# orottier/web-audio-api-rs

Measured on NVIDIA H100. Metric: offline render-quanta/sec (48kHz stereo, 128-frame), higher is better.
Workload: dtype f64 filter state / f32 PCM

## Files before the change

web-audio-api-rs_b200/csrc/wae_kernels.cu:

```cuda
#include "wae_kernels.h"
#include "wae_param_core.h"
#include "wae_param_walk.h"
#include "../../include/wae.h"

#include <algorithm>
#include <cmath>
#include <cstdlib>
#include <vector>
#include <type_traits>
#include <cuda_runtime.h>
#include <math_constants.h>

namespace wae {

#define DEVI __device__ __forceinline__

DEVI float* chan(const BufRef& b, int c, const ChunkInfo& ci) { return b.p + (size_t)c * b.stride + (b.absolute ? ci.f0 : ci.sub); }

DEVI int meta_qi(const ChunkInfo& ci, int n) { return (ci.sub + n) >> 7; }
DEVI bool buf_silent(const BufRef& b, int rows, int qi) {
    if (!b.meta) return false;
    for (int r = 0; r < rows; r++)
        if (!(b.meta[(size_t)r * b.meta_stride + qi] & WAE_META_SILENT)) return false;
    return true;
// ... 3366 lines not shown
    u = cadd(a[2], a[6]); v = csub(a[2], a[6]); a[2] = u; a[6] = cmul(rot16<4>(v, sign), t1);
    u = cadd(a[3], a[7]); v = csub(a[3], a[7]); a[3] = u; a[7] = cmul(rot16<6>(v, sign), t1);
#pragma unroll
    for (int g = 0; g < 8; g += 4) {
        u = cadd(a[g], a[g + 2]); v = csub(a[g], a[g + 2]); a[g] = u; a[g + 2] = cmul(v, t2);
        u = cadd(a[g + 1], a[g + 3]); v = csub(a[g + 1], a[g + 3]); a[g + 1] = u; a[g + 3] = cmul(rot16<4>(v, sign), t2);
    }
#pragma unroll
    for (int m = 0; m < 8; m += 2) {
        u = cadd(a[m], a[m + 1]); v = csub(a[m], a[m + 1]); a[m] = u; a[m + 1] = cmul(v, t3);
    }
}
WAE_HD void bf8_dit(float2 (&a)[8], float2 t1, int sign) {
    const float2 t2 = cmul(t1, t1), t3 = cmul(t2, t2);
    float2 u, v;
#pragma unroll
    for (int m = 0; m < 8; m += 2) {
        v = cmul(a[m + 1], t3); u = a[m]; a[m] = cadd(u, v); a[m + 1] = csub(u, v);
    }
#pragma unroll
    for (int g = 0; g < 8; g += 4) {
        v = cmul(a[g + 2], t2); u = a[g]; a[g] = cadd(u, v); a[g + 2] = csub(u, v);
        v = rot16<4>(cmul(a[g + 3], t2), sign); u = a[g + 1]; a[g + 1] = cadd(u, v); a[g + 3] = csub(u, v);
    }
    v = cmul(a[4], t1); u = a[0]; a[0] = cadd(u, v); a[4] = csub(u, v);
    v = rot16<2>(cmul(a[5], t1), sign); u = a[1]; a[1] = cadd(u, v); a[5] = csub(u, v);
    v = rot16<4>(cmul(a[6], t1), sign); u = a[2]; a[2] = cadd(u, v); a[6] = csub(u, v);
    v = rot16<6>(cmul(a[7], t1), sign); u = a[3]; a[3] = cadd(u, v); a[7] = csub(u, v);
}
WAE_HD void bf16_dif(float2 (&a)[16], int sign) {
    float2 u, v;
#define WAE_BF(i, j, M) u = cadd(a[i], a[j]); v = csub(a[i], a[j]); a[i] = u; a[j] = rot16<M>(v, sign);
    WAE_BF(0, 8, 0) WAE_BF(1, 9, 1) WAE_BF(2, 10, 2) WAE_BF(3, 11, 3) WAE_BF(4, 12, 4) WAE_BF(5, 13, 5) WAE_BF(6, 14, 6) WAE_BF(7, 15, 7)
#pragma unroll
    for (int g = 0; g < 16; g += 8) {
        WAE_BF(g, g + 4, 0) WAE_BF(g + 1, g + 5, 2) WAE_BF(g + 2, g + 6, 4) WAE_BF(g + 3, g + 7, 6)
    }
#pragma unroll
    for (int g = 0; g < 16; g += 4) {
        WAE_BF(g, g + 2, 0) WAE_BF(g + 1, g + 3, 4)
    }
#pragma unroll
    for (int g = 0; g < 16; g += 2) {
        WAE_BF(g, g + 1, 0)
    }
#undef WAE_BF
}
WAE_HD void bf16_dit(float2 (&a)[16], int sign) {
    float2 u, v;
#define WAE_BF(i, j, M) v = rot16<M>(a[j], sign); u = a[i]; a[i] = cadd(u, v); a[j] = csub(u, v);
#pragma unroll
    for (int g = 0; g < 16; g += 2) {
        WAE_BF(g, g + 1, 0)
    }
#pragma unroll
    for (int g = 0; g < 16; g += 4) {
        WAE_BF(g, g + 2, 0) WAE_BF(g + 1, g + 3, 4)
    }
#pragma unroll
    for (int g = 0; g < 16; g += 8) {
        WAE_BF(g, g + 4, 0) WAE_BF(g + 1, g + 5, 2) WAE_BF(g + 2, g + 6, 4) WAE_BF(g + 3, g + 7, 6)
    }
    WAE_BF(0, 8, 0) WAE_BF(1, 9, 1) WAE_BF(2, 10, 2) WAE_BF(3, 11, 3) WAE_BF(4, 12, 4) WAE_BF(5, 13, 5) WAE_BF(6, 14, 6) WAE_BF(7, 15, 7)
#undef WAE_BF
}
struct FftTw { float2 w1, w2, w3; };
static_assert(CV_THREADS == 256 && CV_LOGB == 13, "FftTw assumes 4 radix-8 butterflies per thread and spans 1024 / 128 / 16");
WAE_HD FftTw fft_tw_of(const float2* tw, int t, int sign) {
    FftTw w;
    w.w1 = tw[t << 1];
    w.w2 = tw[(t & 127) << 4];
    w.w3 = tw[(t & 15) << 7];
    if (sign > 0) w.w1.y = -w.w1.y, w.w2.y = -w.w2.y, w.w3.y = -w.w3.y;
    return w;
}
WAE_HD float2 tw_it(float2 w1, int it, int sign) {
    float c, s;
    if (it == 0) return w1;
    if (it == 1) c = 0.98078528040323044913f, s = 0.19509032201612826785f;
    else if (it == 2) c = 0.92387953251128675613f, s = 0.38268343236508977173f;
    else c = 0.83146961230254523708f, s = 0.55557023301960222474f;
    return cmul(w1, make_float2(c, sign > 0 ? s : -s));
}
template <int LOG_Q, bool DIT>
WAE_HD void fft_pass8_one(float2* s, int t, int it, const FftTw& w, int sign) {
    constexpr int q = 1 << LOG_Q;
    const int bf = t + it * CV_THREADS;
    const int lo = bf & (q - 1), hi = bf >> LOG_Q;
    const int base = (hi << (LOG_Q + 3)) + lo;
    float2 a[8];
#pragma unroll
    for (int m = 0; m < 8; m++) a[m] = s[cv_pad(base + m * q)];
    const float2 t1 = LOG_Q == 10 ? tw_it(w.w1, it, sign) : (LOG_Q == 7 ? w.w2 : w.w3);
    if (DIT) bf8_dit(a, t1, sign);
    else bf8_dif(a, t1, sign);
#pragma unroll
    for (int m = 0; m < 8; m++) s[cv_pad(base + m * q)] = a[m];
}
template <bool DIT>
WAE_HD void fft_pass16_one(float2* s, int t, int it, int sign) {
    float2 a[16];
    float2* p = s + cv_pad((t + it * CV_THREADS) * 16);
#pragma unroll
    for (int m = 0; m < 16; m++) a[m] = p[m];
    if (DIT) bf16_dit(a, sign);
    else bf16_dif(a, sign);
#pragma unroll
    for (int m = 0; m < 16; m++) p[m] = a[m];
}
#ifndef WAE_CV_UNROLL
#define WAE_CV_UNROLL 2
#endif
template <int LOG_Q, bool DIT>
DEVI void fft_pass8(float2* s, const FftTw& w, int sign) {
#pragma unroll 1
    for (int i0 = 0; i0 < CV_B / 8 / CV_THREADS; i0 += WAE_CV_UNROLL) {
#pragma unroll
        for (int u = 0; u < WAE_CV_UNROLL; u++) fft_pass8_one<LOG_Q, DIT>(s, threadIdx.x, i0 + u, w, sign);
    }
}
template <bool DIT>
DEVI void fft_pass16(float2* s, int sign) {
#pragma unroll 1
    for (int it = 0; it < CV_B / 16 / CV_THREADS; it++) fft_pass16_one<DIT>(s, threadIdx.x, it, sign);
}
DEVI FftTw fft_tw_load(int sign) { return fft_tw_of(c_tw, threadIdx.x, sign); }
DEVI void fft_dif_smem(float2* s, const FftTw& w) {
    fft_pass8<10, false>(s, w, -1);
    __syncthreads();
    fft_pass8<7, false>(s, w, -1);
    __syncthreads();
    fft_pass8<4, false>(s, w, -1);
    __syncthreads();
    fft_pass16<false>(s, -1);
    __syncthreads();
}
DEVI void fft_dit_smem(float2* s, const FftTw& w) {
    fft_pass16<true>(s, +1);
    __syncthreads();
    fft_pass8<4, true>(s, w, +1);
    __syncthreads();
    fft_pass8<7, true>(s, w, +1);
    __syncthreads();
    fft_pass8<10, true>(s, w, +1);
    __syncthreads();
}
DEVI float2 cv_lane_tw() { return c_tw[cv_brev(threadIdx.x & 31)]; }
DEVI float2 cv_bin_tw(float2 lane_tw, int p) { return cmul(lane_tw, c_rowtw[p >> 5]); }
WAE_HD int cv_mirror(int p) { return cv_brev(CV_B - cv_brev(p)); }
WAE_HD float2 rfft_split(float2 zk, float2 zm, float2 tw) {
    const float2 zc = make_float2(zm.x, -zm.y);
    const float2 e = make_float2(0.5f * (zk.x + zc.x), 0.5f * (zk.y + zc.y));
    const float2 d = make_float2(zk.x - zc.x, zk.y - zc.y);
    const float2 o = make_float2(0.5f * d.y, -0.5f * d.x);
    const float2 r = cmul(tw, o);
    return make_float2(e.x + r.x, e.y + r.y);
}
WAE_HD float2 irfft_merge(float2 yk, float2 ym, float2 tw) {
    const float2 yc = make_float2(ym.x, -ym.y);
    const float2 e = make_float2(yk.x + yc.x, yk.y + yc.y);
    const float2 d = make_float2(yk.x - yc.x, yk.y - yc.y);
    const float2 o = cmul(make_float2(tw.x, -tw.y), d);
    return make_float2(e.x - o.y, e.y + o.x);
}
DEVI void rfft_store(const float2* z, float2* __restrict__ X, float2 lane_tw) {
#pragma unroll 4
    for (int p = threadIdx.x; p < CV_B; p += CV_THREADS) {
        float2 r;
        if (p == 0) {
            const float2 z0 = z[0];
            r = make_float2(z0.x + z0.y, z0.x - z0.y);
        } else {
            r = rfft_split(z[cv_pad(p)], z[cv_pad(cv_mirror(p))], cv_bin_tw(lane_tw, p));
        }
        X[p] = r;
    }
}
DEVI void conv_load_half(float2* z, int c0, const float* __restrict__ src, int valid, const float* __restrict__ src2 = nullptr) {
    const int t = threadIdx.x;
    if (!src || valid <= 0) {
        for (int i = t; i < CV_B / 2; i += CV_THREADS) z[cv_pad(c0 + i)] = make_float2(0.f, 0.f);
    } else if (src2 && ((reinterpret_cast<uintptr_t>(src) | reinterpret_cast<uintptr_t>(src2)) & 15) == 0) {
#pragma unroll 8
        for (int i4 = t; i4 < CV_B / 4; i4 += CV_THREADS) {
            const int n = 4 * i4;
            float4 v = make_float4(0.f, 0.f, 0.f, 0.f);
            if (n + 3 < valid) {
                const float4 a = *reinterpret_cast<const float4*>(src + n), c = *reinterpret_cast<const float4*>(src2 + n);
                v = make_float4(0.5f * (a.x + c.x), 0.5f * (a.y + c.y), 0.5f * (a.z + c.z), 0.5f * (a.w + c.w));
            } else if (n < valid) {
                v.x = 0.5f * (src[n] + src2[n]);
                if (n + 1 < valid) v.y = 0.5f * (src[n + 1] + src2[n + 1]);
                if (n + 2 < valid) v.z = 0.5f * (src[n + 2] + src2[n + 2]);
            }
            float2* d = z + cv_pad(c0 + 2 * i4);
            d[0] = make_float2(v.x, v.y);
            d[1] = make_float2(v.z, v.w);
        }
    } else if (src2) {
        for (int i = t; i < CV_B / 2; i += CV_THREADS) {
            const int n = 2 * i;
            z[cv_pad(c0 + i)] = make_float2(n < valid ? 0.5f * (src[n] + src2[n]) : 0.f, n + 1 < valid ? 0.5f * (src[n + 1] + src2[n + 1]) : 0.f);
        }
    } else if ((reinterpret_cast<uintptr_t>(src) & 15) == 0) {
#pragma unroll 8
        for (int i4 = t; i4 < CV_B / 4; i4 += CV_THREADS) {
            const int n = 4 * i4;
            float4 v = make_float4(0.f, 0.f, 0.f, 0.f);
            if (n + 3 < valid) v = *reinterpret_cast<const float4*>(src + n);
            else if (n < valid) {
                v.x = src[n];
                if (n + 1 < valid) v.y = src[n + 1];
                if (n + 2 < valid) v.z = src[n + 2];
            }
            float2* d = z + cv_pad(c0 + 2 * i4);
            d[0] = make_float2(v.x, v.y);
            d[1] = make_float2(v.z, v.w);
        }
    } else {
        for (int i = t; i < CV_B / 2; i += CV_THREADS) {
            const int n = 2 * i;
            z[cv_pad(c0 + i)] = make_float2(n < valid ? src[n] : 0.f, n + 1 < valid ? src[n + 1] : 0.f);
        }
    }
}

__global__ void __launch_bounds__(CV_THREADS, 3) k_conv_fft_in(const ConvInput* __restrict__ inputs, int n_inputs, ChunkInfo ci) {
    extern __shared__ float2 z[];
    const FftTw w = fft_tw_load(-1);
    const float2 lane_tw = cv_lane_tw();
    const ConvInput ip = inputs[blockIdx.y];
    const int jb = blockIdx.x;
    const int64_t jabs = ci.f0 / CV_B + jb;
    const int64_t to_end = ip.end - (ci.f0 + (int64_t)jb * CV_B);
    if (to_end <= 0) return;
    const bool mix = ip.in_channel < 0;
    const float* in = chan(ip.in, mix ? 0 : ip.in_channel, ci);
    const float* in2 = mix ? chan(ip.in, 1, ci) : nullptr;
    const int64_t left = min((int64_t)ci.nf - (int64_t)jb * CV_B, to_end);
    if (jb == 0) conv_load_half(z, 0, ip.prev, CV_B);
    else conv_load_half(z, 0, in + (size_t)(jb - 1) * CV_B, CV_B, mix ? in2 + (size_t)(jb - 1) * CV_B : nullptr);
    conv_load_half(z, CV_B / 2, in + (size_t)jb * CV_B, (int)(left < CV_B ? left : CV_B), mix ? in2 + (size_t)jb * CV_B : nullptr);
    __syncthreads();
    fft_dif_smem(z, w);
    rfft_store(z, ip.xring + (size_t)(jabs % ip.xring_blocks) * CV_BINS, lane_tw);
}

__global__ void __launch_bounds__(256) k_conv_save_prev(const ConvInput* __restrict__ inputs, int n_inputs, ChunkInfo ci) {
    const ConvInput ip = inputs[blockIdx.y];
    const bool mix = ip.in_channel < 0;
    const float* in = chan(ip.in, mix ? 0 : ip.in_channel, ci);
    const int i = blockIdx.x * blockDim.x + threadIdx.x;
    const int nblocks = (ci.nf + CV_B - 1) / CV_B;
    const int64_t m = (int64_t)(nblocks - 1) * CV_B + i;
    float v = m < ci.nf ? in[m] : 0.f;
    if (mix && m < ci.nf) v = 0.5f * (v + chan(ip.in, 1, ci)[m]);
    ip.prev[i] = v;
}

constexpr int CV_J = 8;
constexpr int CV_MAC_THREADS = 256;
template <bool PACKED, bool FIRST>
DEVI void conv_mac_group(const float2* __restrict__ hp , const float2 (&x)[CV_J], float2 acc[CV_J]) {
    float2 hw[2 * CV_J - 1];
#pragma unroll
    for (int u = FIRST ? CV_J - 1 : 0; u < 2 * CV_J - 1; u++) hw[u] = __ldg(hp + (size_t)u * CV_BINS);
#pragma unroll
    for (int r = 0; r < CV_J; r++) {
#pragma unroll
        for (int jj = FIRST ? r : 0; jj < CV_J; jj++) {
            const float2 h = hw[(CV_J - 1) + jj - r];
            if (PACKED) {
                acc[jj].x = fmaf(h.x, x[r].x, acc[jj].x);
                acc[jj].y = fmaf(h.y, x[r].y, acc[jj].y);
            } else {
                acc[jj].x = fmaf(h.x, x[r].x, fmaf(-h.y, x[r].y, acc[jj].x));
                acc[jj].y = fmaf(h.x, x[r].y, fmaf(h.y, x[r].x, acc[jj].y));
            }
        }
    }
}
template <bool PACKED>
DEVI void conv_mac_bin(const ConvPath& p, const ConvInput& ip, int k, int64_t jabs0, int64_t jabs_last, float2 acc[CV_J]) {
    const int groups = (p.S - 1 + CV_J - 1) / CV_J + 1;
    const int ring = ip.xring_blocks;
    int slot0 = (int)(jabs0 % ring);
    const float2* hp = p.h + k - (ptrdiff_t)(CV_J - 1) * CV_BINS;
    const float2* __restrict__ xr = ip.xring + k;
    int64_t b0 = jabs0;
#pragma unroll 1
    for (int g = 0; g < groups; g++) {
        float2 x[CV_J];
        if (slot0 + CV_J <= ring && b0 >= 0 && b0 + (CV_J - 1) <= jabs_last) {
            const float2* xp = xr + (size_t)slot0 * CV_BINS;
#pragma unroll
            for (int r = 0; r < CV_J; r++) x[r] = __ldg(xp + (size_t)r * CV_BINS);
        } else {
#pragma unroll
            for (int r = 0; r < CV_J; r++) {
                const int64_t bb = b0 + r;
                int slot = slot0 + r;
                while (slot >= ring) slot -= ring;
                x[r] = (bb >= 0 && bb <= jabs_last) ? __ldg(xr + (size_t)slot * CV_BINS) : make_float2(0.f, 0.f);
            }
        }
        if (g == 0) conv_mac_group<PACKED, true>(hp, x, acc);
        else conv_mac_group<PACKED, false>(hp, x, acc);
        hp += (size_t)CV_J * CV_BINS;
        b0 -= CV_J;
        slot0 -= CV_J;
        while (slot0 < 0) slot0 += ring;
    }
}
#ifndef WAE_CV_MAC_MINB
#define WAE_CV_MAC_MINB 3
#endif
__global__ void __launch_bounds__(CV_MAC_THREADS, WAE_CV_MAC_MINB) k_conv_mac(const ConvPath* __restrict__ paths, const ConvInput* __restrict__ inputs, int n_paths,
                                                             ChunkInfo ci) {
    const ConvPath p = paths[blockIdx.y];
    if (p.S == 1) return;
    const ConvInput ip = inputs[p.input];
    const int nb = (ci.nf + CV_B - 1) / CV_B;
    constexpr int TILES = CV_B / CV_MAC_THREADS;
    const int k = (blockIdx.x % TILES) * CV_MAC_THREADS + threadIdx.x;
    const int j0 = (blockIdx.x / TILES) * CV_J;
    if (ci.f0 + (int64_t)j0 * CV_B >= p.end) return;
    const int64_t jabs0 = ci.f0 / CV_B + j0;
    const int64_t jabs_last = ci.f0 / CV_B + nb - 1;
    float2 acc[CV_J];
#pragma unroll
    for (int jj = 0; jj < CV_J; jj++) acc[jj] = make_float2(0.f, 0.f);
    if (k == 0) conv_mac_bin<true>(p, ip, k, jabs0, jabs_last, acc);
    else conv_mac_bin<false>(p, ip, k, jabs0, jabs_last, acc);
#pragma unroll
    for (int jj = 0; jj < CV_J; jj++)
        if (j0 + jj < nb) p.y[(size_t)(j0 + jj) * CV_BINS + k] = acc[jj];
}

__global__ void __launch_bounds__(CV_THREADS, 3) k_conv_ifft(const ConvPath* __restrict__ paths, const ConvInput* __restrict__ inputs, int n_paths, ChunkInfo ci) {
    extern __shared__ float2 z[];
    const FftTw w = fft_tw_load(+1);
    const float2 lane_tw = cv_lane_tw();
    const ConvPath p = paths[blockIdx.y];
    const int jb = blockIdx.x;
    if (ci.f0 + (int64_t)jb * CV_B >= p.end) return;
    const float2* __restrict__ Y = p.y + (size_t)jb * CV_BINS;
    const int t = threadIdx.x;
    if (p.S == 1) {
        const ConvInput ip = inputs[p.input];
        const int64_t jabs = ci.f0 / CV_B + jb;
        const float2* __restrict__ X = ip.xring + (size_t)(jabs % ip.xring_blocks) * CV_BINS;
        const float2* __restrict__ H = p.h;
        auto prod = [&](int q) {
            const float2 h = __ldg(H + q), x = __ldg(X + q);
            return make_float2(fmaf(h.x, x.x, __fmul_rn(-h.y, x.y)), fmaf(h.x, x.y, __fmul_rn(h.y, x.x)));
        };
#pragma unroll 4
        for (int q = t; q < CV_B; q += CV_THREADS) {
            float2 yk, ym;
            if (q == 0) {
                const float2 h = __ldg(H), x = __ldg(X);
                yk = make_float2(h.x * x.x, 0.f);
                ym = make_float2(h.y * x.y, 0.f);
            } else {
                yk = prod(q);
                ym = prod(cv_mirror(q));
            }
            z[cv_pad(q)] = irfft_merge(yk, ym, cv_bin_tw(lane_tw, q));
        }
    } else {
#pragma unroll 4
    for (int q = t; q < CV_B; q += CV_THREADS) {
        float2 yk, ym;
        if (q == 0) {
            const float2 y0 = Y[0];
            yk = make_float2(y0.x, 0.f);
            ym = make_float2(y0.y, 0.f);
        } else {
            yk = Y[q];
            ym = Y[cv_mirror(q)];
        }
        z[cv_pad(q)] = irfft_merge(yk, ym, cv_bin_tw(lane_tw, q));
    }
    }
    __syncthreads();
    fft_dit_smem(z, w);
    const float scale = 1.f / (float)(2 * CV_B);
    float* out = chan(p.out, p.out_channel, ci) + (size_t)jb * CV_B;
    int64_t left = (int64_t)ci.nf - (int64_t)jb * CV_B;
    if (p.limit >= 0 && p.limit - (ci.f0 + (int64_t)jb * CV_B) < left) left = p.limit - (ci.f0 + (int64_t)jb * CV_B);
    const int valid = (int)(left < CV_B ? (left > 0 ? left : 0) : CV_B);
    if ((reinterpret_cast<uintptr_t>(out) & 15) == 0) {
#pragma unroll 4
        for (int i4 = t; i4 < CV_B / 4; i4 += CV_THREADS) {
            const int n = 4 * i4;
            const float2* c = z + cv_pad(CV_B / 2 + 2 * i4);
            float4 v = make_float4(c[0].x * scale, c[0].y * scale, c[1].x * scale, c[1].y * scale);
            if (n + 3 < valid) {
                float4* dst = reinterpret_cast<float4*>(out + n);
                if (p.accumulate) {
                    const float4 o = *dst;
                    v.x += o.x, v.y += o.y, v.z += o.z, v.w += o.w;
                }
                *dst = v;
            } else {
                const float vv[4] = {v.x, v.y, v.z, v.w};
#pragma unroll
                for (int u = 0; u < 4; u++)
                    if (n + u < valid) out[n + u] = p.accumulate ? out[n + u] + vv[u] : vv[u];
            }
        }
    } else {
        for (int i = t; i < CV_B / 2; i += CV_THREADS) {
            const int n = 2 * i;
            const float2 c = z[cv_pad(CV_B / 2 + i)];
            if (n < valid) out[n] = p.accumulate ? out[n] + c.x * scale : c.x * scale;
            if (n + 1 < valid) out[n + 1] = p.accumulate ? out[n + 1] + c.y * scale : c.y * scale;
        }
    }
}


__global__ void __launch_bounds__(128) k_conv_cmp_map(const ConvCmpInst* __restrict__ insts, int n_inst, ChunkInfo ci) {
    const int ii = blockIdx.x * 4 + (threadIdx.x >> 5);
    if (ii >= n_inst) return;
    const int lane = threadIdx.x & 31;
    const ConvCmpInst& p = insts[ii];
    const int nq = ci.nf / 128;
    int n_proc = 0;
    for (int q0 = 0; q0 < nq; q0 += 32) {
        const int q = q0 + lane;
        bool fed = false;
        if (q < nq) {
            const int qi = meta_qi(ci, q * 128);
            fed = !buf_silent(p.in, p.in_ch, qi) && buf_count(p.in, p.in_ch, qi) >= 2;
        }
        const unsigned m = __ballot_sync(0xffffffffu, fed);
        if (fed) p.qmap[n_proc + __popc(m & ((1u << lane) - 1u))] = q;
        n_proc += __popc(m);
    }
    if (lane == 0) {
        const int64_t c0 = *p.cursor;
        p.wdesc[0] = c0;
        p.wdesc[1] = (int64_t)n_proc * 128;
        *p.cursor = c0 + (int64_t)n_proc * 128;
    }
}
__global__ void __launch_bounds__(256) k_conv_cmp_gather(const ConvCmpInst* __restrict__ insts, ChunkInfo ci) {
    const ConvCmpInst& p = insts[blockIdx.y];
    const int64_t c0 = p.wdesc[0], n_new = p.wdesc[1];
    const int64_t w = (int64_t)blockIdx.x * 256 + threadIdx.x;
    const int64_t carried = CV_B + c0 % CV_B;
    float v = 0.f;
    if (w < carried) {
        v = p.carry[w];
    } else if (w - carried < n_new) {
        const int k = (int)(w - carried);
        v = chan(p.in, 1, ci)[p.qmap[k >> 7] * 128 + (k & 127)];
    }
    p.win[w] = v;
}
__global__ void __launch_bounds__(CV_THREADS, 3) k_conv_cmp_fft(const ConvCmpInst* __restrict__ insts, ChunkInfo ci) {
    extern __shared__ float2 z[];
    const ConvCmpInst& p = insts[blockIdx.y];
    const int64_t c0 = p.wdesc[0], c1 = c0 + p.wdesc[1];
    const int jb = blockIdx.x;
    const int64_t j = c0 / CV_B + jb;
    if (c1 == c0 || j * CV_B >= c1) return;
    const FftTw w = fft_tw_load(-1);
    const float2 lane_tw = cv_lane_tw();
    const float* win = p.win + (size_t)jb * CV_B;
    const int64_t left = c1 - j * CV_B;
    conv_load_half(z, 0, win, CV_B);
    conv_load_half(z, CV_B / 2, win + CV_B, (int)(left < CV_B ? left : CV_B));
    __syncthreads();
    fft_dif_smem(z, w);
    rfft_store(z, p.x.xring + (size_t)(j % p.x.xring_blocks) * CV_BINS, lane_tw);
}
__global__ void __launch_bounds__(256) k_conv_cmp_carry(const ConvCmpInst* __restrict__ insts) {
    const ConvCmpInst& p = insts[blockIdx.y];
    const int64_t c0 = p.wdesc[0], c1 = c0 + p.wdesc[1];
    const int64_t first = (c1 / CV_B - c0 / CV_B) * CV_B;
    const int i = blockIdx.x * 256 + threadIdx.x;
    p.carry[i] = p.win[first + i];
}
__global__ void __launch_bounds__(CV_MAC_THREADS, WAE_CV_MAC_MINB) k_conv_cmp_mac(const ConvCmpInst* __restrict__ insts, ChunkInfo ci) {
    const int64_t c0 = insts[blockIdx.y].wdesc[0], c1 = c0 + insts[blockIdx.y].wdesc[1];
    if (c1 == c0) return;
    const int64_t jfirst = c0 / CV_B, jlast = (c1 - 1) / CV_B;
    constexpr int TILES = CV_B / CV_MAC_THREADS;
    const int k = (blockIdx.x % TILES) * CV_MAC_THREADS + threadIdx.x;
    const int j0 = (blockIdx.x / TILES) * CV_J;
    if (jfirst + j0 > jlast) return;
    const ConvPath path = insts[blockIdx.y].path;
    const ConvInput x = insts[blockIdx.y].x;
    float2 acc[CV_J];
#pragma unroll
    for (int jj = 0; jj < CV_J; jj++) acc[jj] = make_float2(0.f, 0.f);
    if (k == 0) conv_mac_bin<true>(path, x, k, jfirst + j0, jlast, acc);
    else conv_mac_bin<false>(path, x, k, jfirst + j0, jlast, acc);
#pragma unroll
    for (int jj = 0; jj < CV_J; jj++)
        if (jfirst + j0 + jj <= jlast) path.y[(size_t)(j0 + jj) * CV_BINS + k] = acc[jj];
}
__global__ void __launch_bounds__(CV_THREADS, 3) k_conv_cmp_ifft(const ConvCmpInst* __restrict__ insts, ChunkInfo ci) {
    extern __shared__ float2 z[];
    const ConvCmpInst& p = insts[blockIdx.y];
    const int64_t c0 = p.wdesc[0], c1 = c0 + p.wdesc[1];
    const int jb = blockIdx.x;
    const int64_t j = c0 / CV_B + jb;
    if (c1 == c0 || j * CV_B >= c1) return;
    const FftTw w = fft_tw_load(+1);
    const float2 lane_tw = cv_lane_tw();
    const float2* __restrict__ Y = p.path.y + (size_t)jb * CV_BINS;
    const int t = threadIdx.x;
#pragma unroll 4
    for (int q = t; q < CV_B; q += CV_THREADS) {
        float2 yk, ym;
        if (q == 0) {
            const float2 y0 = Y[0];
            yk = make_float2(y0.x, 0.f);
            ym = make_float2(y0.y, 0.f);
        } else {
            yk = Y[q];
            ym = Y[cv_mirror(q)];
        }
        z[cv_pad(q)] = irfft_merge(yk, ym, cv_bin_tw(lane_tw, q));
    }
    __syncthreads();
    fft_dit_smem(z, w);
    const float scale = 1.f / (float)(2 * CV_B);
    float* out = chan(p.path.out, p.path.out_channel, ci);
    const int64_t b0 = j * CV_B;
    const int lo = (int)((c0 > b0 ? c0 : b0) - b0), hi = (int)((c1 < b0 + CV_B ? c1 : b0 + CV_B) - b0);
    for (int i = lo + t; i < hi; i += CV_THREADS) {
        const float2 c = z[cv_pad(CV_B / 2 + (i >> 1))];
        const int k = (int)(b0 + i - c0);
        out[p.qmap[k >> 7] * 128 + (k & 127)] = ((i & 1) ? c.y : c.x) * scale;
    }
}

__global__ void __launch_bounds__(CV_THREADS) k_conv_ir_fft(const float* __restrict__ ir, int64_t ir_len, int64_t ir_stride, float2* __restrict__ h,
                                                            int S) {
    extern __shared__ float2 z[];
    const FftTw w = fft_tw_load(-1);
    const float2 lane_tw = cv_lane_tw();
    const int seg = blockIdx.x, c = blockIdx.y;
    const float* src = ir + (size_t)c * ir_stride + (size_t)seg * CV_B;
    const int64_t left = ir_len - (int64_t)seg * CV_B;
    conv_load_half(z, 0, src, (int)(left < CV_B ? left : CV_B));
    conv_load_half(z, CV_B / 2, nullptr, 0);
    __syncthreads();
    fft_dif_smem(z, w);
    rfft_store(z, h + ((size_t)c * (S + WAE_CONV_H_PAD) + WAE_CONV_H_PAD_LO + seg) * CV_BINS, lane_tw);
}


constexpr int RB_TILE = 1024;
__global__ void __launch_bounds__(256) k_resp_power(RespBindItem* __restrict__ items) {
    __shared__ float buf[2][4][RB_TILE + 1];
    __shared__ float part[4];
    RespBindItem& it = items[blockIdx.x];
    if (!it.normalize) return;
    const int ch = it.channels, t = threadIdx.x, warp = t >> 5;
    const int64_t len = it.len;
    const int64_t ntiles = (len + RB_TILE - 1) / RB_TILE;
    auto load = [&](int64_t tile, int b, int t0, int nt) {
        const int64_t f0 = tile * RB_TILE;
        const int cnt = (int)(len - f0 < RB_TILE ? len - f0 : RB_TILE);
        for (int k = t - t0; k < ch * RB_TILE; k += nt) {
            const int c = k / RB_TILE, i = k % RB_TILE;
            if (i < cnt) buf[b][c][i] = __ldcs(it.src + (int64_t)c * it.src_stride + f0 + i);
        }
    };
    load(0, 0, 0, blockDim.x);
    __syncthreads();
    float s = 0.f;
    for (int64_t tile = 0; tile < ntiles; tile++) {
        if (warp != 0) {
            if (tile + 1 < ntiles) load(tile + 1, (int)((tile + 1) & 1), 32, blockDim.x - 32);
        } else if (t < ch) {
            const float* __restrict__ x = buf[tile & 1][t];
            const int cnt = (int)(len - tile * RB_TILE < RB_TILE ? len - tile * RB_TILE : RB_TILE);
#pragma unroll 16
            for (int i = 0; i < cnt; i++) s = __fadd_rn(s, __fmul_rn(x[i], x[i]));
        }
        __syncthreads();
    }
    if (t < ch) part[t] = s;
    __syncthreads();
    if (t == 0) {
        float power = 0.f;
        for (int c = 0; c < ch; c++) power = __fadd_rn(power, part[c]);
        power = __fsqrt_rn(__fdiv_rn(power, (float)((uint64_t)ch * (uint64_t)len)));
        if (!isfinite(power) || power < 0.000125f) power = 0.000125f;
        float scale = __fdiv_rn(1.f, power);
        scale = __fmul_rn(scale, 0.00125f);
        scale = __fmul_rn(scale, __fdiv_rn(44100.f, it.sample_rate));
        if (ch == 4) scale = __fmul_rn(scale, 0.5f);
        it.scale = scale;
    }
}

__global__ void __launch_bounds__(256) k_resp_trim(RespBindItem* __restrict__ items) {
    RespBindItem& it = items[blockIdx.y];
    const int c = blockIdx.z;
    if (c >= it.channels) return;
    const float* __restrict__ src = it.src + (int64_t)c * it.src_stride;
    const float scale = it.scale;
    int best = 0;
    for (int64_t i = (int64_t)blockIdx.x * blockDim.x + threadIdx.x; i < it.len; i += (int64_t)gridDim.x * blockDim.x)
        if (!(fabsf(__fmul_rn(__ldg(src + i), scale)) < 0.000001f)) best = (int)(i + 1);
    best = __reduce_max_sync(0xffffffffu, best);
    if ((threadIdx.x & 31) == 0 && best > 0) atomicMax(&it.m[c], best);
}

__global__ void __launch_bounds__(CV_THREADS) k_resp_fft(const RespBindItem* __restrict__ items) {
    extern __shared__ float2 z[];
    const RespBindItem& it = items[blockIdx.z];
    const int seg = blockIdx.x, c = blockIdx.y;
    if (seg >= it.S || c >= it.channels) return;
    const FftTw w = fft_tw_load(-1);
// ... 191 lines not shown
                const bool aligned = start <= clock.block_time(q) && offset == 0.;
                const AbsnStart st = absn_start(clock, start, stop);
                r->s.n_first = st.n_first;
                r->s.n_stop = st.n_stop;
                r->start_delta = st.t_first - st.start;
                r->n_start = q * 128;
                r->fast_end = absn_fast_end(clock, p.lq, q * 128, p.duration);
                r->fast_ok = aligned && p.flag && stop > 1e300;
                if (bind_offset) r->offset = bound_offset;
                if (bind_duration) r->s.duration = bound_duration;
                break;
            }
            case SCHED_ABSN_SERIAL: {
                AbsnSerialInst* r = reinterpret_cast<AbsnSerialInst*>(d);
                r->start_time = start;
                r->stop_time = stop;
                if (bind_offset) r->offset = bound_offset;
                if (bind_duration) r->duration = bound_duration;
                break;
            }
        }
    }
}

__global__ void __launch_bounds__(128) k_bind_loops(const LoopBindItem* __restrict__ items, int n_items) {
    const int i = blockIdx.x * blockDim.x + threadIdx.x;
    if (i >= n_items) return;
    const LoopBindItem it = items[i];
    const double ls = sched_clamp(it.points[0], it.lo[0], it.hi[0]);
    const double le = sched_clamp(it.points[1], it.lo[1], it.hi[1]);
    for (int k = 0; k < it.n_patches; k++) {
        const LoopPatch p = it.patches[k];
        const AbsnLoopPoints lp = absn_loop_points(ls, le, p.buffer_duration);
        if (p.kind == LOOP_BOUND) {
            AbsnBoundInst* r = static_cast<AbsnBoundInst*>(p.dst);
            r->s.loop_start = lp.actual_start;
            r->s.loop_end = lp.actual_end;
        } else {
            AbsnSerialInst* r = static_cast<AbsnSerialInst*>(p.dst);
            r->loop_start = lp.start;
            r->loop_end = lp.end;
        }
    }
}

__global__ void __launch_bounds__(128) k_absn_loop_schedule(const LoopWalk* __restrict__ walks, int n, int* overflow) {
    const int i = blockIdx.x * blockDim.x + threadIdx.x;
    if (i >= n) return;
    const LoopWalk w = walks[i];
    AbsnBoundInst& r = *w.rec;
    const AbsnSlowInst& o = r.s;
    const double computed_rate = (double)r.rate * exp2((double)r.detune / 1200.);
    const AbsnSlowDerived d = absn_slow_derive(r.dt, computed_rate, r.offset, r.start_delta, o.buffer_duration, o.duration, true, o.loop_end,
                                               o.n_first, o.n_stop);
    const int64_t n_end = o.n_stop < w.lq ? o.n_stop : w.lq;
    int32_t k = absn_loop_segments(o.loop_start, o.loop_end, d.step, o.n_first, n_end, d.offset0, const_cast<int64_t*>(o.seg_n),
                                   const_cast<double*>(o.seg_bt), w.cap);
    if (k < 0) {
        atomicExch(overflow, 1);
        k = w.cap;
    }
    r.s.n_seg = k;
}

__global__ void __launch_bounds__(128) k_bind_output(const OutPatch* __restrict__ entries, int n, float* base) {
    const int i = blockIdx.x * blockDim.x + threadIdx.x;
    if (i >= n) return;
    const OutPatch e = entries[i];
    *e.dst = base + e.off;
}

static void host_twiddles() {
    if (h_tw[0].x == 1.f) return;
    for (int k = 0; k < CV_B; k++) {
        const double a = -2.0 * 3.14159265358979323846 * (double)k / (2.0 * CV_B);
        h_tw[k] = make_float2((float)std::cos(a), (float)std::sin(a));
    }
}
static int brev8(int r) {
    int o = 0;
    for (int b = 0; b < 8; b++) o |= ((r >> b) & 1) << (7 - b);
    return o;
}
template <int LOG_Q, bool DIT>
static void host_pass8(float2* s, int sign) {
    for (int t = 0; t < CV_THREADS; t++) {
        const FftTw w = fft_tw_of(h_tw, t, sign);
        for (int it = 0; it < CV_B / 8 / CV_THREADS; it++) fft_pass8_one<LOG_Q, DIT>(s, t, it, w, sign);
    }
}
template <bool DIT>
static void host_pass16(float2* s, int sign) {
    for (int t = 0; t < CV_THREADS; t++)
        for (int it = 0; it < CV_B / 16 / CV_THREADS; it++) fft_pass16_one<DIT>(s, t, it, sign);
}
static void host_fft(float2* s, bool inverse) {
    if (!inverse) {
        host_pass8<10, false>(s, -1), host_pass8<7, false>(s, -1), host_pass8<4, false>(s, -1), host_pass16<false>(s, -1);
    } else {
        host_pass16<true>(s, +1), host_pass8<4, true>(s, +1), host_pass8<7, true>(s, +1), host_pass8<10, true>(s, +1);
    }
}
void conv_fft_selftest(float* data, int mode) {
    host_twiddles();
    std::vector<float2> s(CV_SMEM_ELEMS), x(CV_B);
    float2* io = reinterpret_cast<float2*>(data);
    auto bin_tw = [](int p) { return cmul(h_tw[cv_brev(p & 31)], h_tw[brev8(p >> 5)]); };
    if (mode == 0 || mode == 1) {
        for (int i = 0; i < CV_B; i++) s[cv_pad(i)] = io[i];
        host_fft(s.data(), mode == 1);
        for (int i = 0; i < CV_B; i++) io[i] = s[cv_pad(i)];
    } else if (mode == 2) {
        for (int i = 0; i < CV_B; i++) s[cv_pad(i)] = io[i];
        host_fft(s.data(), false);
        for (int p = 0; p < CV_B; p++) {
            if (p == 0) io[0] = make_float2(s[0].x + s[0].y, s[0].x - s[0].y);
            else x[p] = rfft_split(s[cv_pad(p)], s[cv_pad(cv_mirror(p))], bin_tw(p));
        }
        for (int p = 1; p < CV_B; p++) io[p] = x[p];
    } else {
        for (int p = 0; p < CV_B; p++) {
            const float2 yk = p == 0 ? make_float2(io[0].x, 0.f) : io[p];
            const float2 ym = p == 0 ? make_float2(io[0].y, 0.f) : io[cv_mirror(p)];
            s[cv_pad(p)] = irfft_merge(yk, ym, bin_tw(p));
        }
        host_fft(s.data(), true);
        const float scale = 1.f / (float)(2 * CV_B);
        for (int i = 0; i < CV_B; i++) io[i] = make_float2(s[cv_pad(i)].x * scale, s[cv_pad(i)].y * scale);
    }
}
void upload_twiddles() {
    host_twiddles();
    float2 row[CV_ROWS];
    for (int r = 0; r < CV_ROWS; r++) row[r] = h_tw[brev8(r)];
    cudaMemcpyToSymbol(c_tw, h_tw, sizeof(float2) * CV_B);
    cudaMemcpyToSymbol(c_rowtw, row, sizeof(row));
}

__global__ void __launch_bounds__(256) k_analyser_fft(const float* __restrict__ ring, uint32_t write_index, int fft_size, float smoothing,
                                                      float* __restrict__ last_fft, float* __restrict__ out_db) {
    extern __shared__ float2 zf[];
    const int RING = 32768 + 128;
    const int n = fft_size / 2;
    const int t = threadIdx.x;
    const float PI32 = 3.14159265358979323846f;
    int bits = 0;
    while ((1 << bits) < n) bits++;
    for (int i = t; i < n; i += blockDim.x) {
        float v[2];
        for (int h = 0; h < 2; h++) {
            int idx = 2 * i + h;
            float x = ring[(RING + write_index - fft_size + idx) % RING];
            float w = 0.42f - 0.5f * cosf(2.f * PI32 * (float)idx / (float)fft_size) + 0.08f * cosf(4.f * PI32 * (float)idx / (float)fft_size);
            v[h] = x * w;
        }
        int r = (int)(__brev((unsigned)i) >> (32 - bits));
        zf[bits == 0 ? 0 : r] = make_float2(v[0], v[1]);
    }
    __syncthreads();
    for (int len = 2; len <= n; len <<= 1) {
        const int half = len >> 1;
        for (int b = t; b < n / 2; b += blockDim.x) {
            int grp = b / half, j = b % half;
            int i0 = grp * len + j, i1 = i0 + half;
            float sn, cs;
            sincospif(-2.f * (float)j / (float)len, &sn, &cs);
            float2 u = zf[i0], x = zf[i1];
            float2 v = make_float2(x.x * cs - x.y * sn, x.x * sn + x.y * cs);
            zf[i0] = make_float2(u.x + v.x, u.y + v.y);
            zf[i1] = make_float2(u.x - v.x, u.y - v.y);
        }
        __syncthreads();
    }
    const float norm = 1.f / (float)fft_size;
    for (int k = t; k < n; k += blockDim.x) {
        float2 X;
        if (k == 0) {
            X = make_float2(zf[0].x + zf[0].y, 0.f);
        } else {
            float2 zk = zf[k], zc = make_float2(zf[n - k].x, -zf[n - k].y);
            float2 e = make_float2(0.5f * (zk.x + zc.x), 0.5f * (zk.y + zc.y));
            float2 d = make_float2(zk.x - zc.x, zk.y - zc.y);
            float2 o = make_float2(0.5f * d.y, -0.5f * d.x);
            float sn, cs;
            sincospif(-2.f * (float)k / (float)fft_size, &sn, &cs);
            X = make_float2(e.x + (o.x * cs - o.y * sn), e.y + (o.x * sn + o.y * cs));
        }
        float mag = hypotf(X.x, X.y) * norm;
        float value = smoothing * last_fft[k] + (1.f - smoothing) * mag;
        if (!isfinite(value)) value = 0.f;
        last_fft[k] = value;
        out_db[k] = 20.f * log10f(value);
    }
}

__global__ void __launch_bounds__(256) k_resample_linear(const float* __restrict__ in, int64_t len, float* __restrict__ out, int64_t target_len) {
    int64_t i = (int64_t)blockIdx.x * blockDim.x + threadIdx.x;
    if (i >= target_len) return;
    double position = (double)i / (double)(target_len - 1);
    double playhead = position * (double)(len - 1);
    double fl = floor(playhead);
    int64_t prev = (int64_t)fl;
    int64_t next = prev + 1 < len - 1 ? prev + 1 : len - 1;
    float k = (float)(playhead - fl);
    out[i] = __fadd_rn(__fmul_rn(1.f - k, in[prev]), __fmul_rn(k, in[next]));
}

__global__ void __launch_bounds__(256) k_bind_sources(const BindItem* __restrict__ items, int n) {
    const int c = blockIdx.z;
    for (int i = blockIdx.y; i < n; i += gridDim.y) {
        const BindItem it = items[i];
// ... 453 lines not shown
```

Before: 1.375 billion.

## Fuse inverse-FFT final pass with output store and drop redundant syncs in convolution

Generalizes the radix-8 FFT pass over load/store functors so the last DIT pass of the convolver inverse FFT writes scaled output samples directly to global memory. Only the second half of the frame, the overlap-save valid part, is stored, which removes the trailing __syncthreads and the separate smem-to-global copy loop. The spectrum merge is remapped so each warp writes exactly the shared-memory rows its first radix-16 pass reads, letting a __syncwarp replace a block-wide barrier. The cost is that output stores become 8-byte scattered writes instead of float4-vectorized coalesced stores. The host selftest is reworked to use the same fused store path.

```diff
diff --git a/web-audio-api-rs_b200/csrc/wae_kernels.cu b/web-audio-api-rs_b200/csrc/wae_kernels.cu
--- a/web-audio-api-rs_b200/csrc/wae_kernels.cu
+++ b/web-audio-api-rs_b200/csrc/wae_kernels.cu
@@ -3472,20 +3472,30 @@
     else c = 0.83146961230254523708f, s = 0.55557023301960222474f;
     return cmul(w1, make_float2(c, sign > 0 ? s : -s));
 }
-template <int LOG_Q, bool DIT>
-WAE_HD void fft_pass8_one(float2* s, int t, int it, const FftTw& w, int sign) {
+template <int LOG_Q, bool DIT, class Load, class Store>
+WAE_HD void fft_pass8_io(int t, int it, const FftTw& w, int sign, const Load& load, const Store& store) {
     constexpr int q = 1 << LOG_Q;
     const int bf = t + it * CV_THREADS;
     const int lo = bf & (q - 1), hi = bf >> LOG_Q;
     const int base = (hi << (LOG_Q + 3)) + lo;
     float2 a[8];
 #pragma unroll
-    for (int m = 0; m < 8; m++) a[m] = s[cv_pad(base + m * q)];
+    for (int m = 0; m < 8; m++) a[m] = load(m, base + m * q);
     const float2 t1 = LOG_Q == 10 ? tw_it(w.w1, it, sign) : (LOG_Q == 7 ? w.w2 : w.w3);
     if (DIT) bf8_dit(a, t1, sign);
     else bf8_dif(a, t1, sign);
 #pragma unroll
-    for (int m = 0; m < 8; m++) s[cv_pad(base + m * q)] = a[m];
+    for (int m = 0; m < 8; m++) store(m, base + m * q, a[m]);
+}
+struct SmemIo {
+    float2* s;
+    WAE_HD float2 operator()(int, int e) const { return s[cv_pad(e)]; }
+    WAE_HD void operator()(int, int e, float2 v) const { s[cv_pad(e)] = v; }
+};
+template <int LOG_Q, bool DIT>
+WAE_HD void fft_pass8_one(float2* s, int t, int it, const FftTw& w, int sign) {
+    const SmemIo io{s};
+    fft_pass8_io<LOG_Q, DIT>(t, it, w, sign, io, io);
 }
 template <bool DIT>
 WAE_HD void fft_pass16_one(float2* s, int t, int it, int sign) {
@@ -3501,13 +3511,17 @@
 #ifndef WAE_CV_UNROLL
 #define WAE_CV_UNROLL 2
 #endif
+template <int LOG_Q, bool DIT, class Load, class Store>
+DEVI void fft_pass8(const FftTw& w, int sign, const Load& load, const Store& store) {
+#pragma unroll 1
+    for (int i0 = 0; i0 < CV_B / 8 / CV_THREADS; i0 += WAE_CV_UNROLL) {
+#pragma unroll
+        for (int u = 0; u < WAE_CV_UNROLL; u++) fft_pass8_io<LOG_Q, DIT>(threadIdx.x, i0 + u, w, sign, load, store);
+    }
+}
 template <int LOG_Q, bool DIT>
 DEVI void fft_pass8(float2* s, const FftTw& w, int sign) {
-#pragma unroll 1
-    for (int i0 = 0; i0 < CV_B / 8 / CV_THREADS; i0 += WAE_CV_UNROLL) {
-#pragma unroll
-        for (int u = 0; u < WAE_CV_UNROLL; u++) fft_pass8_one<LOG_Q, DIT>(s, threadIdx.x, i0 + u, w, sign);
-    }
+    fft_pass8<LOG_Q, DIT>(w, sign, SmemIo{s}, SmemIo{s});
 }
 template <bool DIT>
 DEVI void fft_pass16(float2* s, int sign) {
@@ -3523,16 +3537,6 @@
     fft_pass8<4, false>(s, w, -1);
     __syncthreads();
     fft_pass16<false>(s, -1);
-    __syncthreads();
-}
-DEVI void fft_dit_smem(float2* s, const FftTw& w) {
-    fft_pass16<true>(s, +1);
-    __syncthreads();
-    fft_pass8<4, true>(s, w, +1);
-    __syncthreads();
-    fft_pass8<7, true>(s, w, +1);
-    __syncthreads();
-    fft_pass8<10, true>(s, w, +1);
     __syncthreads();
 }
 DEVI float2 cv_lane_tw() { return c_tw[cv_brev(threadIdx.x & 31)]; }
@@ -3614,6 +3618,60 @@
         }
     }
 }
+struct ConvOut {
+    float* out;
+    int valid;
+    bool accumulate;
+    WAE_HD void operator()(int n, float2 v) const {
+        const float scale = 1.f / (float)(2 * CV_B);
+        v = make_float2(v.x * scale, v.y * scale);
+        if ((reinterpret_cast<uintptr_t>(out) & 7) == 0 && n + 1 < valid) {
+            float2* d = reinterpret_cast<float2*>(out + n);
+            if (accumulate) {
+                const float2 o = *d;
+                v.x += o.x, v.y += o.y;
+            }
+            *d = v;
+        } else {
+            if (n < valid) out[n] = accumulate ? out[n] + v.x : v.x;
+            if (n + 1 < valid) out[n + 1] = accumulate ? out[n + 1] + v.y : v.y;
+        }
+    }
+};
+template <class Spec, class Store>
+DEVI void fft_dit(float2* s, const FftTw& w, float2 lane_tw, const Spec& spec, const Store& store) {
+    const int t = threadIdx.x;
+#pragma unroll 4
+    for (int k = 0; k < CV_B / CV_THREADS; k++) {
+        const int q = 512 * ((t >> 5) + (CV_THREADS / 32) * (k >> 4)) + 32 * (k & 15) + (t & 31);
+        float2 yk, ym;
+        spec(q, yk, ym);
+        s[cv_pad(q)] = irfft_merge(yk, ym, cv_bin_tw(lane_tw, q));
+    }
+    __syncwarp();
+    fft_pass16<true>(s, +1);
+    __syncthreads();
+    fft_pass8<4, true>(s, w, +1);
+    __syncthreads();
+    fft_pass8<7, true>(s, w, +1);
+    __syncthreads();
+    fft_pass8<10, true>(w, +1, SmemIo{s}, [&](int m, int e, float2 v) {
+        if (m >= 4) store(2 * (e - CV_B / 2), v);
+    });
+}
+struct ConvSpec {
+    const float2* __restrict__ Y;
+    DEVI void operator()(int q, float2& yk, float2& ym) const {
+        if (q == 0) {
+            const float2 y0 = Y[0];
+            yk = make_float2(y0.x, 0.f);
+            ym = make_float2(y0.y, 0.f);
+        } else {
+            yk = Y[q];
+            ym = Y[cv_mirror(q)];
+        }
+    }
+};
 
 __global__ void __launch_bounds__(CV_THREADS, 3) k_conv_fft_in(const ConvInput* __restrict__ inputs, int n_inputs, ChunkInfo ci) {
     extern __shared__ float2 z[];
@@ -3734,8 +3792,9 @@
     const ConvPath p = paths[blockIdx.y];
     const int jb = blockIdx.x;
     if (ci.f0 + (int64_t)jb * CV_B >= p.end) return;
-    const float2* __restrict__ Y = p.y + (size_t)jb * CV_BINS;
-    const int t = threadIdx.x;
+    int64_t left = (int64_t)ci.nf - (int64_t)jb * CV_B;
+    if (p.limit >= 0 && p.limit - (ci.f0 + (int64_t)jb * CV_B) < left) left = p.limit - (ci.f0 + (int64_t)jb * CV_B);
+    const ConvOut out{chan(p.out, p.out_channel, ci) + (size_t)jb * CV_B, (int)(left < CV_B ? (left > 0 ? left : 0) : CV_B), p.accumulate != 0};
     if (p.S == 1) {
         const ConvInput ip = inputs[p.input];
         const int64_t jabs = ci.f0 / CV_B + jb;
@@ -3745,9 +3804,7 @@
             const float2 h = __ldg(H + q), x = __ldg(X + q);
             return make_float2(fmaf(h.x, x.x, __fmul_rn(-h.y, x.y)), fmaf(h.x, x.y, __fmul_rn(h.y, x.x)));
         };
-#pragma unroll 4
-        for (int q = t; q < CV_B; q += CV_THREADS) {
-            float2 yk, ym;
+        fft_dit(z, w, lane_tw, [&](int q, float2& yk, float2& ym) {
             if (q == 0) {
                 const float2 h = __ldg(H), x = __ldg(X);
                 yk = make_float2(h.x * x.x, 0.f);
@@ -3756,57 +3813,9 @@
                 yk = prod(q);
                 ym = prod(cv_mirror(q));
             }
-            z[cv_pad(q)] = irfft_merge(yk, ym, cv_bin_tw(lane_tw, q));
-        }
+        }, out);
     } else {
-#pragma unroll 4
-    for (int q = t; q < CV_B; q += CV_THREADS) {
-        float2 yk, ym;
-        if (q == 0) {
-            const float2 y0 = Y[0];
-            yk = make_float2(y0.x, 0.f);
-            ym = make_float2(y0.y, 0.f);
-        } else {
-            yk = Y[q];
-            ym = Y[cv_mirror(q)];
-        }
-        z[cv_pad(q)] = irfft_merge(yk, ym, cv_bin_tw(lane_tw, q));
-    }
-    }
-    __syncthreads();
-    fft_dit_smem(z, w);
-    const float scale = 1.f / (float)(2 * CV_B);
-    float* out = chan(p.out, p.out_channel, ci) + (size_t)jb * CV_B;
-    int64_t left = (int64_t)ci.nf - (int64_t)jb * CV_B;
-    if (p.limit >= 0 && p.limit - (ci.f0 + (int64_t)jb * CV_B) < left) left = p.limit - (ci.f0 + (int64_t)jb * CV_B);
-    const int valid = (int)(left < CV_B ? (left > 0 ? left : 0) : CV_B);
-    if ((reinterpret_cast<uintptr_t>(out) & 15) == 0) {
-#pragma unroll 4
-        for (int i4 = t; i4 < CV_B / 4; i4 += CV_THREADS) {
-            const int n = 4 * i4;
-            const float2* c = z + cv_pad(CV_B / 2 + 2 * i4);
-            float4 v = make_float4(c[0].x * scale, c[0].y * scale, c[1].x * scale, c[1].y * scale);
-            if (n + 3 < valid) {
-                float4* dst = reinterpret_cast<float4*>(out + n);
-                if (p.accumulate) {
-                    const float4 o = *dst;
-                    v.x += o.x, v.y += o.y, v.z += o.z, v.w += o.w;
-                }
-                *dst = v;
-            } else {
-                const float vv[4] = {v.x, v.y, v.z, v.w};
-#pragma unroll
-                for (int u = 0; u < 4; u++)
-                    if (n + u < valid) out[n + u] = p.accumulate ? out[n + u] + vv[u] : vv[u];
-            }
-        }
-    } else {
-        for (int i = t; i < CV_B / 2; i += CV_THREADS) {
-            const int n = 2 * i;
-            const float2 c = z[cv_pad(CV_B / 2 + i)];
-            if (n < valid) out[n] = p.accumulate ? out[n] + c.x * scale : c.x * scale;
-            if (n + 1 < valid) out[n + 1] = p.accumulate ? out[n + 1] + c.y * scale : c.y * scale;
-        }
+        fft_dit(z, w, lane_tw, ConvSpec{p.y + (size_t)jb * CV_BINS}, out);
     }
 }
 
@@ -3902,32 +3911,20 @@
     if (c1 == c0 || j * CV_B >= c1) return;
     const FftTw w = fft_tw_load(+1);
     const float2 lane_tw = cv_lane_tw();
-    const float2* __restrict__ Y = p.path.y + (size_t)jb * CV_BINS;
-    const int t = threadIdx.x;
-#pragma unroll 4
-    for (int q = t; q < CV_B; q += CV_THREADS) {
-        float2 yk, ym;
-        if (q == 0) {
-            const float2 y0 = Y[0];
-            yk = make_float2(y0.x, 0.f);
-            ym = make_float2(y0.y, 0.f);
-        } else {
-            yk = Y[q];
-            ym = Y[cv_mirror(q)];
-        }
-        z[cv_pad(q)] = irfft_merge(yk, ym, cv_bin_tw(lane_tw, q));
-    }
-    __syncthreads();
-    fft_dit_smem(z, w);
     const float scale = 1.f / (float)(2 * CV_B);
     float* out = chan(p.path.out, p.path.out_channel, ci);
     const int64_t b0 = j * CV_B;
     const int lo = (int)((c0 > b0 ? c0 : b0) - b0), hi = (int)((c1 < b0 + CV_B ? c1 : b0 + CV_B) - b0);
-    for (int i = lo + t; i < hi; i += CV_THREADS) {
-        const float2 c = z[cv_pad(CV_B / 2 + (i >> 1))];
+    const int* __restrict__ qmap = p.qmap;
+    auto put = [&](int i, float v) {
+        if (i < lo || i >= hi) return;
         const int k = (int)(b0 + i - c0);
-        out[p.qmap[k >> 7] * 128 + (k & 127)] = ((i & 1) ? c.y : c.x) * scale;
-    }
+        out[qmap[k >> 7] * 128 + (k & 127)] = v * scale;
+    };
+    fft_dit(z, w, lane_tw, ConvSpec{p.path.y + (size_t)jb * CV_BINS}, [&](int n, float2 v) {
+        put(n, v.x);
+        put(n + 1, v.y);
+    });
 }
 
 __global__ void __launch_bounds__(CV_THREADS) k_conv_ir_fft(const float* __restrict__ ir, int64_t ir_len, int64_t ir_stride, float2* __restrict__ h,
@@ -4285,25 +4282,35 @@
     for (int b = 0; b < 8; b++) o |= ((r >> b) & 1) << (7 - b);
     return o;
 }
+template <int LOG_Q, bool DIT, class Load, class Store>
+static void host_pass8(const Load& load, const Store& store, int sign) {
+    for (int t = 0; t < CV_THREADS; t++) {
+        const FftTw w = fft_tw_of(h_tw, t, sign);
+        for (int it = 0; it < CV_B / 8 / CV_THREADS; it++) fft_pass8_io<LOG_Q, DIT>(t, it, w, sign, load, store);
+    }
+}
 template <int LOG_Q, bool DIT>
 static void host_pass8(float2* s, int sign) {
-    for (int t = 0; t < CV_THREADS; t++) {
-        const FftTw w = fft_tw_of(h_tw, t, sign);
-        for (int it = 0; it < CV_B / 8 / CV_THREADS; it++) fft_pass8_one<LOG_Q, DIT>(s, t, it, w, sign);
-    }
+    host_pass8<LOG_Q, DIT>(SmemIo{s}, SmemIo{s}, sign);
 }
 template <bool DIT>
 static void host_pass16(float2* s, int sign) {
     for (int t = 0; t < CV_THREADS; t++)
         for (int it = 0; it < CV_B / 16 / CV_THREADS; it++) fft_pass16_one<DIT>(s, t, it, sign);
 }
-static void host_fft(float2* s, bool inverse) {
-    if (!inverse) {
-        host_pass8<10, false>(s, -1), host_pass8<7, false>(s, -1), host_pass8<4, false>(s, -1), host_pass16<false>(s, -1);
-    } else {
-        host_pass16<true>(s, +1), host_pass8<4, true>(s, +1), host_pass8<7, true>(s, +1), host_pass8<10, true>(s, +1);
-    }
-}
+static void host_fft_forward(float2* s) {
+    host_pass8<10, false>(s, -1), host_pass8<7, false>(s, -1), host_pass8<4, false>(s, -1), host_pass16<false>(s, -1);
+}
+static void host_dit_head(float2* s) { host_pass16<true>(s, +1), host_pass8<4, true>(s, +1), host_pass8<7, true>(s, +1); }
+struct HostFrameStore {
+    float2* io;
+    ConvOut second;
+    WAE_HD void operator()(int m, int e, float2 v) const {
+        const float scale = 1.f / (float)(2 * CV_B);
+        if (m < 4) io[e] = make_float2(v.x * scale, v.y * scale);
+        else second(2 * (e - CV_B / 2), v);
+    }
+};
 void conv_fft_selftest(float* data, int mode) {
     host_twiddles();
     std::vector<float2> s(CV_SMEM_ELEMS), x(CV_B);
@@ -4311,11 +4318,12 @@
     auto bin_tw = [](int p) { return cmul(h_tw[cv_brev(p & 31)], h_tw[brev8(p >> 5)]); };
     if (mode == 0 || mode == 1) {
         for (int i = 0; i < CV_B; i++) s[cv_pad(i)] = io[i];
-        host_fft(s.data(), mode == 1);
+        if (mode == 0) host_fft_forward(s.data());
+        else host_dit_head(s.data()), host_pass8<10, true>(s.data(), +1);
         for (int i = 0; i < CV_B; i++) io[i] = s[cv_pad(i)];
     } else if (mode == 2) {
         for (int i = 0; i < CV_B; i++) s[cv_pad(i)] = io[i];
-        host_fft(s.data(), false);
+        host_fft_forward(s.data());
         for (int p = 0; p < CV_B; p++) {
             if (p == 0) io[0] = make_float2(s[0].x + s[0].y, s[0].x - s[0].y);
             else x[p] = rfft_split(s[cv_pad(p)], s[cv_pad(cv_mirror(p))], bin_tw(p));
@@ -4327,9 +4335,8 @@
             const float2 ym = p == 0 ? make_float2(io[0].y, 0.f) : io[cv_mirror(p)];
             s[cv_pad(p)] = irfft_merge(yk, ym, bin_tw(p));
         }
-        host_fft(s.data(), true);
-        const float scale = 1.f / (float)(2 * CV_B);
-        for (int i = 0; i < CV_B; i++) io[i] = make_float2(s[cv_pad(i)].x * scale, s[cv_pad(i)].y * scale);
+        host_dit_head(s.data());
+        host_pass8<10, true>(SmemIo{s.data()}, HostFrameStore{io, ConvOut{data + CV_B, CV_B, false}}, +1);
     }
 }
 void upload_twiddles() {
```

Result: no change. 1.374 billion (median of 6 runs) (-0.0%).
